# Ameek94/BOBE

Measured on AMD Instinct MI355X. Metric: GP fit+acquisition cycles/sec at N=4096 d=8, 65536 cands; Cholesky GF/s, higher is better.
Workload: dtype f64

## Files before the change

bobe_amd/csrc/chol_kernels.hpp:

```cpp
#pragma once
#include "kernels_common.hpp"

namespace bobe {

constexpr int PLD = 130;
constexpr int POTF2_DLD = 17;

template <bool LOWER = false, int NWAVES = 4>
__device__ __forceinline__ void block_load(double* S, const double* __restrict__ G, int64_t ld) {
  const int lane = threadIdx.x & 63, wave = threadIdx.x >> 6;
  constexpr int NI = TILE / NWAVES;
  v2d v[NI];
#pragma unroll
  for (int i = 0; i < NI; ++i) {
    const int r = NWAVES * i + wave;
    const int c = LOWER ? ((2 * lane <= r) ? 2 * lane : (r & ~1)) : 2 * lane;
    v[i] = *reinterpret_cast<const v2d*>(G + (int64_t)r * ld + c);
  }
#pragma unroll
  for (int i = 0; i < NI; ++i) *reinterpret_cast<v2d*>(S + (NWAVES * i + wave) * PLD + 2 * lane) = v[i];
}
__device__ __forceinline__ void block_store_lower(const double* S, double* __restrict__ G, int64_t ld) {
  const int lane = threadIdx.x & 63, wave = threadIdx.x >> 6;
#pragma unroll 8
// ... 305 lines not shown
          for (int ks = 0; ks < 4; ++ks) {
            const double av = S[(16 * i + (lane & 15)) * PLD + 16 * k + 4 * ks + (lane >> 4)];
            const double bv = S[(16 * k + 4 * ks + (lane >> 4)) * PLD + 16 * j + (lane & 15)];
            tacc = __builtin_amdgcn_mfma_f64_16x16x4f64(av, bv, tacc, 0, 0, 0);
          }
        }
        v4d racc = (v4d){0.0, 0.0, 0.0, 0.0};
#pragma unroll
        for (int r = 0; r < 4; ++r) {
          const double av = -S[(16 * i + (lane & 15)) * PLD + 16 * i + (lane >> 4) + 4 * r];
          racc = __builtin_amdgcn_mfma_f64_16x16x4f64(av, tacc[r], racc, 0, 0, 0);
        }
        if (slot == 0) res0 = racc; else res1 = racc;
      }
    }
    __syncthreads();
#pragma unroll
    for (int slot = 0; slot < 2; ++slot) {
      const int j = wave + 4 * slot;
      if (j < i) {
        const v4d racc = slot == 0 ? res0 : res1;
#pragma unroll
        for (int r = 0; r < 4; ++r) S[(16 * i + (lane >> 4) + 4 * r) * PLD + 16 * j + (lane & 15)] = racc[r];
      }
    }
    __syncthreads();
  }
  block_store_lower(S, Ib, ldl);
}

__global__ __launch_bounds__(256) void k_trti_diag(double* __restrict__ L, int64_t lda,
                                                   double* __restrict__ Linv, int64_t ldl, int64_t bsA = 0,
                                                   int64_t bsL = 0, const double* __restrict__ diag = nullptr,
                                                   int64_t bsD = 0, int first_aside = 1 << 30) {
  extern __shared__ double S[];
  const int blk = blockIdx.x;
  L += blockIdx.y * bsA;
  Linv += blockIdx.y * bsL;
  double* Lb = L + ((int64_t)blk * TILE) * lda + (int64_t)blk * TILE;
  double* Ib = Linv + ((int64_t)blk * TILE) * ldl + (int64_t)blk * TILE;
  if (diag && blk >= first_aside) {
    block_load(S, diag + blockIdx.y * bsD + (int64_t)blk * TILE * TILE, TILE);
    __syncthreads();
    block_store_lower(S, Lb, lda);
  } else {
    block_load(S, Lb, lda);
  }
  __syncthreads();
  trti_block(S, Ib, ldl);
}

constexpr int TRSM_DLD = 17;
constexpr int TRSM_SMEM_BYTES = (TILE * PLD + 8 * 16 * TRSM_DLD) * 8;
__global__ __launch_bounds__(256) void k_trsm_panel(double* __restrict__ A, int64_t lda,
                                                    const double* __restrict__ Dinv, int64_t ldl, int k,
                                                    int64_t bsA = 0, int64_t bsL = 0) {
  extern __shared__ double S[];
  A += blockIdx.y * bsA;
  Dinv += blockIdx.y * bsL;
  double* D = S + TILE * PLD;
  const int t = threadIdx.x, lane = t & 63, wave = t >> 6;
  const int64_t row0 = (int64_t)(k + 1) * TILE + (int64_t)blockIdx.x * 64 + wave * 16;
  const int64_t col0 = (int64_t)k * TILE;
  const double* Lkk = A + col0 * lda + col0;
  const double* Dk = Dinv + col0 * ldl + col0;
  const int g = lane >> 4, li = lane & 15;
  double* Aw = A + row0 * lda + col0;
  double* Sw = S + (wave * 16) * PLD;
  v2d xr[16], lr[32];
// ... 464 lines not shown
```

bobe_amd/csrc/gp_consumers.hip:

```cpp
#include "gp_handle.hpp"

#include "consumer_kernels.hpp"

using namespace bobe;

namespace bobe {
void configure_consumer_kernels() {
  static bool done[64] = {false};
  if (!first_use_on_device(done)) return;
  for_each_kern_dcap([](auto KE, auto DC) {
    allow_big_lds((k_hmc_run<KE, DC>), CHAIN_LDS_BYTES);
    allow_big_lds((k_rwalk<KE, DC>), CHAIN_LDS_BYTES);
    allow_big_lds((k_nuts_run<KE, DC>), NUTS_LDS_BYTES);
  });
}
}

void bobe_gp::set_gate(const double* sv, int64_t n_sv, const double* dual, double intercept, double gamma, double threshold,
                       double minus_inf) {
  use();
  sync();
  if (!sv || n_sv <= 0) {
    gate = Gate{nullptr, nullptr, 0, 0, 0.0, 0.0, threshold, minus_inf, GATE_NONE, nullptr, nullptr, 0.0, 0.0};
    return;
// ... 395 lines not shown
  not_pd = src.not_pd;
}

void bobe_gp::release_all() {
  (void)hipSetDevice(device);
  if (stream) (void)hipStreamSynchronize(stream);
  DBuf* bufs[] = {&X, &y, &XsT, &A, &Linv, &Tmp, &alpha, &w, &part, &gpart, &res, &info, &probs, &diag, &in_stage, &z_stage, &CsT, &ZsT, &kXC, &kXZ, &VZ, &WZ, &basez, &sc, &qpart, &pv,
                  &ps, &o_mean, &o_var, &o_wipv, &o_wipstd, &o_misc, &kin_a, &kin_b, &kout, &wg_ws, &gate_sv, &gate_dual, &gate_ell, &ell_ws, &ell_perm,
                  &vxc, &vxc2, &loo_ws};
  for (DBuf* b : bufs) b->release();
  for (auto& pr : prof_events) {
    (void)hipEventDestroy(pr.first);
    (void)hipEventDestroy(pr.second);
  }
  if (h_res) (void)hipHostFree(h_res);
  if (h_in) (void)hipHostFree(h_in);
  h_in = nullptr;
  for (hipStream_t st : slot_streams) {
    (void)hipStreamSynchronize(st);
    (void)hipStreamDestroy(st);
  }
  own.release();
  batch.release();
  for (EvalWs* sl : slots) {
    sl->release();
    delete sl;
  }
  slots.clear();
  for (auto& kv : chol_plans) {
    kv.second.d_jobs.release();
    kv.second.d_colk0.release();
  }
  if (ev_batch) (void)hipEventDestroy(ev_batch);
  if (own_stream && stream) (void)hipStreamDestroy(stream);
}
```

bobe_amd/csrc/gp_factor.hip:

```cpp
#include "gp_handle.hpp"

#include <chrono>

#include "chol_kernels.hpp"

using namespace bobe;

namespace bobe {

constexpr int SYRK32_BK = 128, SYRK64_BK = 16;
constexpr int SYRK32_SMEM = gemm_smem_doubles_exact<KC, KC, 32, 32, SYRK32_BK>() * 8 / 2;
constexpr int SYRK64_SMEM = gemm_smem_doubles_exact<KC, KC, 64, 64, SYRK64_BK>() * 8;

void configure_factor_kernels() {
  static bool done[64] = {false};
  if (!first_use_on_device(done)) return;
  allow_big_lds(k_potf2<true>, POTF2_SMEM_BYTES);
  allow_big_lds(k_potf2<false>, POTF2_SMEM_BYTES);
  allow_big_lds(k_trti_diag, POTF2_SMEM_BYTES);
  allow_big_lds(k_trsm_panel, TRSM_SMEM_BYTES);
  allow_big_lds((k_chol_panel<false, 3>), POTF2_SMEM_BYTES);
  allow_big_lds((k_chol_panel<false, 4>), POTF2_SMEM_BYTES);
  allow_big_lds((k_chol_panel<true, 3>), POTF2_SMEM_BYTES);
  allow_big_lds((k_chol_panel<true, 4>), POTF2_SMEM_BYTES);
  allow_big_lds(k_trtri_T<128>, GEMM_SMEM_BYTES);
  allow_big_lds(k_trtri_R<128>, GEMM_SMEM_BYTES);
  allow_big_lds(k_syrk_trail<64, SYRK64_BK>, SYRK64_SMEM);
  allow_big_lds(k_syrk_trail<64, SYRK64_BK, true>, SYRK64_SMEM);
  allow_big_lds(k_syrk_trail<32, SYRK32_BK>, SYRK32_SMEM);
  allow_big_lds(k_trtri_T<64>, GEMM64_SMEM_BYTES);
  allow_big_lds(k_trtri_R<64>, GEMM64_SMEM_BYTES);
  allow_big_lds(k_trtri_T<64, true>, GEMM64_SMEM_BYTES);
  allow_big_lds(k_trtri_R<64, true>, GEMM64_SMEM_BYTES);
  allow_big_lds(k_trtri_T<32>, GEMM32_SMEM_BYTES);
  allow_big_lds(k_trtri_R<32>, GEMM32_SMEM_BYTES);
  allow_big_lds(k_lauum_tiles32, GEMM32_SMEM_BYTES);
  for_each_kern_dcap([](auto KE, auto DC) {
    allow_big_lds((k_lauum_grad<KE, DC, 64>), GEMM64_SMEM_BYTES);
    allow_big_lds((k_lauum_grad<KE, DC, 64, true>), GEMM64_SMEM_BYTES);
    allow_big_lds((k_lauum_grad<KE, DC, 128>), GEMM_SMEM_BYTES);
  });
}

const Tuning& tuning() {
  static Tuning t = [] {
    Tuning v{512, 600, 300, 1, BOBE_MAX_MLL_SLOTS, 2048, 1, 1, false, false, true, true, true};
    auto geti = [](const char* name, int& dst) {
      const char* e = std::getenv(name);
      if (e) dst = std::atoi(e);
      return e != nullptr;
    };
    geti("BOBE_SYRK32_BELOW", v.syrk32_below);
    geti("BOBE_TRTRI64", v.trtri64_below);
    geti("BOBE_PAIR_MIN", v.pair_min);
    geti("BOBE_LOCKSTEP_MIN_N", v.lockstep_min_n);
    v.mll_slots_set = geti("BOBE_MLL_SLOTS", v.mll_slots);
    geti("BOBE_GRAPH_MAX_N", v.graph_max_n);
    geti("BOBE_XCD_SHARES", v.xcd_shares);
    geti("BOBE_FILL", v.fill);
    v.trace = std::getenv("BOBE_TRACE") != nullptr;
    int reuse = 1;
    geti("BOBE_FACTOR_REUSE", reuse);
    v.factor_reuse = reuse != 0;
    int glds = 1;
    geti("BOBE_GEMM_GLDS", glds);
    v.gemm_glds = glds != 0;
    int glds64 = 1;
    geti("BOBE_GEMM64_GLDS", glds64);
    v.gemm64_glds = glds64 != 0;
    return v;
  }();
  return t;
}

double default_refine_kappa() {
  static const double v = [] {
    const char* e = std::getenv("BOBE_REFINE_KAPPA");
    return e ? std::atof(e) : 1e6;
  }();
  return v;
}

int default_solve_block() {
  static const int v = [] {
    const char* e = std::getenv("BOBE_SOLVE_BLOCK");
    const int b = e ? std::atoi(e) : TILE;
    return b > 0 ? (b + TILE - 1) / TILE * TILE : TILE;
  }();
  return v;
}

int default_solve_panel() {
  static const int v = [] {
    const char* e = std::getenv("BOBE_SOLVE_PANEL");
    const int b = e ? std::atoi(e) : 512;
    return b > 0 ? (b + TILE - 1) / TILE * TILE : 512;
  }();
  return v;
}

int64_t default_solve_chunk() {
  static const int64_t v = [] {
    const char* e = std::getenv("BOBE_SOLVE_CHUNK");
    const int64_t c = e ? std::atoll(e) : 32768;
    return c > 0 ? (c + TILE - 1) / TILE * TILE : 0;
  }();
  return v;
}

double default_pivot_floor_ulp() {
  static const double v = [] {
    const char* e = std::getenv("BOBE_PIVOT_FLOOR_ULP");
    if (!e) return 0.0;
    const double u = std::atof(e);
    return u >= 0.0 ? u : 0.0;
  }();
  return v;
}

}

void bobe_gp::build_probs() {
  struct Item { int depth, lo, mid, hi; };
  std::vector<Item> items;
  struct Rec {
    static void go(std::vector<Item>& it, int depth, int lo, int hi) {
      if (hi - lo <= 1) return;
      const int mid = lo + (hi - lo) / 2;
      it.push_back({depth, lo, mid, hi});
      go(it, depth + 1, lo, mid);
      go(it, depth + 1, mid, hi);
    }
  };
  Rec::go(items, 0, 0, nb);
  int maxd = -1;
  for (auto& i : items) maxd = i.depth > maxd ? i.depth : maxd;
  std::vector<TriProb> flat;
  depths.clear();
  for (int dd = 0; dd <= maxd; ++dd) {
    Depth D{(int)flat.size(), 0, 0};
    for (auto& i : items)
      if (i.depth == dd) {
        flat.push_back({i.lo, i.mid, i.hi, D.nblocks});
        D.nblocks += (i.hi - i.mid) * (i.mid - i.lo);
        D.count++;
      }
    depths.push_back(D);
  }
  if (!flat.empty()) {
    probs.ensure(flat.size() * sizeof(TriProb));
    HIPCHK(hipMemcpy(probs.p, flat.data(), flat.size() * sizeof(TriProb), hipMemcpyHostToDevice));
  }
}

void bobe_gp::alloc_for_n() {
  own.ensure(*this, 1);
  const size_t mat = (size_t)Np * Np * sizeof(double);
  const size_t vec = (size_t)Np * sizeof(double);
  A.ensure(mat);
  Linv.ensure(mat);
  Tmp.ensure(mat);
  y.ensure(vec);
  alpha.ensure(vec);
  w.ensure(vec);
  XsT.ensure((size_t)d * vec);
  const int64_t pw = Np > chunk ? Np : chunk;
  part.ensure((size_t)nb * pw * sizeof(double));
  gpart.ensure((size_t)own.gps() * sizeof(double));
  res.ensure(128 * sizeof(double));
  info.ensure(sizeof(int));
  diag.ensure((size_t)nb * TILE * TILE * sizeof(double));
  build_probs();
  build_plans();
  forget_evals();
}

void bobe_gp::EvalWs::ensure(const bobe_gp& g, int B) {
  if (!h_res) {
    HIPCHK(hipHostMalloc(reinterpret_cast<void**>(&h_res), (size_t)width * (128 * sizeof(double) + sizeof(Hyper)),
                         hipHostMallocDefault));
    h_hyp = reinterpret_cast<Hyper*>(h_res + (size_t)width * 128);
  }
  if (B > cap || g.Np != Np) {
    for (bobe::EvalTag& t : tag) t.clear();
// ... 193 lines not shown
    for (int f = 1; f < nb; ++f) {
      const auto dc = build(f, nullptr);
      if (dc.first > 0 && dc.second * FILL_SLACK <= dc.first) { far = f; break; }
    }
  }
  CholPlan& pl = chol_plans[key];
  build(far, &pl);
  for (const FillJob& j : pl.jobs)
    if (!(j.ti >= j.tj && j.ti < 2 * nb && j.tj >= 0 && j.k0 >= 0 && j.k1 > j.k0 && j.k1 <= j.tj - (j.tj & 1)))
      throw Err(BOBE_ERR_STATE, "internal error: filler job outside the matrix");
  if (!pl.jobs.empty()) {
    pl.d_jobs.ensure(pl.jobs.size() * sizeof(FillJob));
    HIPCHK(hipMemcpy(pl.d_jobs.p, pl.jobs.data(), pl.jobs.size() * sizeof(FillJob), hipMemcpyHostToDevice));
  }
  bool need_tab = false;
  for (const CholOp& op : pl.ops) need_tab = need_tab || (op.kind != 0 && !op.uniform);
  if (need_tab) {
    pl.d_colk0.ensure(pl.colk0.size() * sizeof(int));
    HIPCHK(hipMemcpy(pl.d_colk0.p, pl.colk0.data(), pl.colk0.size() * sizeof(int), hipMemcpyHostToDevice));
  }
  if (tu.trace)
    std::fprintf(stderr, "[bobe] chol plan nb=%d B=%d fill=%d: deferred columns from %d, %lld of %lld tile-panels in fillers, "
                 "%lld caught up (%zu jobs)\n", nb, B, (int)fill, pl.far_start, (long long)pl.deferred_units,
                 (long long)pl.total_units, (long long)pl.catchup_units, pl.jobs.size());
  return pl;
}

void bobe_gp::build_plans() {
  if (nb <= 0) return;
  (void)chol_plan(1, false);
  if (fill_pays(1)) (void)chol_plan(1, true);
}

void bobe_gp::potrf(double* a, double* linv, int* info_dev, int B, int64_t bsA, int64_t bsL, double* dg, bool defer_diag) {
  if (!dg) dg = diag.d();
  const int64_t bsD = (int64_t)nb * TILE * TILE;
  int first_aside = nb;
  const CholPlan& pl = chol_plan(B, fill_pays(B));
  const FillJob* jobs = static_cast<const FillJob*>(pl.d_jobs.p);
  const int* coltab = static_cast<const int*>(pl.d_colk0.p);
  for (const CholOp& op : pl.ops) {
    if (op.kind == 0) {
      const int kk = op.k;
      const int rr = nb - 1 - kk;
      const int strips = panel_strips(B, rr);
      const int np_ = panel_workgroups(rr, strips);
      const int rows_below = rr * TILE;
      const int nv = (int)std::min<int64_t>(TILE, N - (int64_t)kk * TILE);
      if (B * np_ <= std::max(num_cus, 1)) {
        first_aside = std::min(first_aside, kk);
        prof_begin(BOBE_PROF_POTF2);
#define PANEL_LAUNCH(FILLV, GRIDX, ...)                                                                                        \
  do {                                                                                                                         \
    if (strips == 3)                                                                                                           \
      hipLaunchKernelGGL((k_chol_panel<FILLV, 3>), dim3(GRIDX, B), dim3(PANEL_THREADS), POTF2_SMEM_BYTES, stream, a, Np, bsA, \
                         linv, Np, bsL, kk, np_, info_dev, nv, dg, bsD, __VA_ARGS__);                                          \
    else                                                                                                                       \
      hipLaunchKernelGGL((k_chol_panel<FILLV, 4>), dim3(GRIDX, B), dim3(PANEL_THREADS), POTF2_SMEM_BYTES, stream, a, Np, bsA, \
                         linv, Np, bsL, kk, np_, info_dev, nv, dg, bsD, __VA_ARGS__);                                          \
  } while (0)
        if (op.tab_cnt > 0) PANEL_LAUNCH(true, np_ + op.tab_cnt / 2, jobs + op.tab_off, op.tab_cnt, rows_below);
        else PANEL_LAUNCH(false, np_, (const FillJob*)nullptr, 0, rows_below);
#undef PANEL_LAUNCH
        prof_end(BOBE_PROF_POTF2);
      } else {
        prof_begin(BOBE_PROF_POTF2);
        hipLaunchKernelGGL(k_potf2<true>, dim3(B), dim3(256), POTF2_SMEM_BYTES, stream, a, Np, linv, Np, kk, info_dev, nv, bsA,
                           bsL);
        prof_end(BOBE_PROF_POTF2);
        if (rr > 0) {
          prof_begin(BOBE_PROF_TRSM);
          hipLaunchKernelGGL(k_trsm_panel, dim3(2 * rr, B), dim3(256), TRSM_SMEM_BYTES, stream, a, Np, (const double*)linv, Np,
                             kk, bsA, bsL);
          prof_end(BOBE_PROF_TRSM);
        }
      }
    } else {
      prof_begin(BOBE_PROF_SYRK);
      if (op.uniform) {
        syrk(a, op.k0_min, op.k, op.first, op.kind == 1 ? 1 : 0, B, bsA);
      } else {
        const int ncols = op.last_active - op.first + 1;
        const bool few = ncols <= 8 && ncols < nb - op.first;
        syrk(a, op.k0_plain, op.k, op.first, few ? 2 : 0, B, bsA, coltab + op.tab_off, pl.far_start, few ? ncols : 0);
      }
      prof_end(BOBE_PROF_SYRK);
    }
  }
  cur->aside_first = 1 << 30;
  cur->aside_dg = nullptr;
  if (first_aside < nb) {
    if (defer_diag) {
      cur->aside_first = first_aside;
      cur->aside_dg = dg;
    } else {
      hipLaunchKernelGGL(k_copy_diag, dim3(nb - first_aside, B), dim3(256), 0, stream, a, Np, bsA, (const double*)dg, bsD,
                         first_aside);
    }
  }
  LAUNCH_CHECK();
}

void bobe_gp::trtri(double* a, double* linv, double* tmp, int B, int64_t bsA, int64_t bsL, int64_t bsT) {
  const Tuning& tu = tuning();
  prof_begin(BOBE_PROF_TRTRI);
  hipLaunchKernelGGL(k_trti_diag, dim3(nb, B), dim3(256), POTF2_SMEM_BYTES, stream, a, Np, linv, Np, bsA, bsL, cur->aside_dg,
                     (int64_t)nb * TILE * TILE, cur->aside_first);
  cur->aside_first = 1 << 30;
  cur->aside_dg = nullptr;
  prof_end(BOBE_PROF_TRTRI);
  for (int dd = (int)depths.size() - 1; dd >= 0; --dd) {
    const Depth& D = depths[dd];
    const TriProb* pr = static_cast<const TriProb*>(probs.p) + D.first;
    prof_begin(BOBE_PROF_TRTRI);
    if (B * 2 * D.nblocks <= std::max(num_cus, 1)) {
      const TileGrid tg = tile_grid(8 * D.nblocks);
      hipLaunchKernelGGL(k_trtri_T<32>, dim3(tg.grid, B), dim3(256), GEMM32_SMEM_BYTES, stream, a, Np,
                         (const double*)linv, Np, tmp, Np, pr, D.count, bsA, bsL, bsT, tg.per);
      hipLaunchKernelGGL(k_trtri_R<32>, dim3(tg.grid, B), dim3(256), GEMM32_SMEM_BYTES, stream, linv, Np,
                         (const double*)tmp, Np, pr, D.count, bsL, bsT, tg.per);
    } else if (D.nblocks < tu.trtri64_below) {
      const TileGrid tg = tile_grid(2 * D.nblocks);
      const auto kT = tu.gemm64_glds ? k_trtri_T<64, true> : k_trtri_T<64, false>;
      const auto kR = tu.gemm64_glds ? k_trtri_R<64, true> : k_trtri_R<64, false>;
      hipLaunchKernelGGL(kT, dim3(tg.grid, B), dim3(256), GEMM64_SMEM_BYTES, stream, a, Np,
                         (const double*)linv, Np, tmp, Np, pr, D.count, bsA, bsL, bsT, tg.per);
      hipLaunchKernelGGL(kR, dim3(tg.grid, B), dim3(256), GEMM64_SMEM_BYTES, stream, linv, Np,
                         (const double*)tmp, Np, pr, D.count, bsL, bsT, tg.per);
    } else {
      hipLaunchKernelGGL(k_trtri_T<128>, dim3(D.nblocks, B), dim3(256), GEMM_SMEM_BYTES, stream, a, Np,
                         (const double*)linv, Np, tmp, Np, pr, D.count, bsA, bsL, bsT);
      hipLaunchKernelGGL(k_trtri_R<128>, dim3(D.nblocks, B), dim3(256), GEMM_SMEM_BYTES, stream, linv, Np,
                         (const double*)tmp, Np, pr, D.count, bsL, bsT);
    }
    prof_end(BOBE_PROF_TRTRI);
  }
  LAUNCH_CHECK();
}

int bobe_gp::lauum(const Hyper& h, const double* linv, const double* al, const double* xst, double* kinv_out,
                   const Hyper* hdev, double* gp_out, int B, int64_t bsL, int64_t bsV, int64_t bsX, int64_t bsP,
                   double* scratch, int64_t bsS, int64_t bsKout) {
  const LauumTiling t = lauum_tiling(nb);
  const int ntiles = t.ntiles;
  double* gpo = gp_out ? gp_out : gpart.d();
  const bool split = t.small && scratch && !kinv_out && B * ntiles < 4 * std::max(num_cus, 1);
  double* kio = split ? scratch : kinv_out;
  const int64_t bsK = split ? bsS : bsKout;
  prof_begin(BOBE_PROF_LAUUM);
  if (split) {
    hipLaunchKernelGGL(k_lauum_tiles32, dim3(4 * ntiles * B), dim3(256), GEMM32_SMEM_BYTES, stream, linv, Np, Np, scratch, Np,
                       bsL, bsS, B);
  }
  with_lauum_variant(h.kern, h.d, t, [&](auto KE, auto DC, auto TT, auto GL) {
    hipLaunchKernelGGL((k_lauum_grad<KE, DC, TT, GL>), dim3(ntiles * B), dim3(256),
                       (TT == 128 ? GEMM_SMEM_BYTES : GEMM64_SMEM_BYTES), stream, linv, Np, Np, N, al, xst, Np, h, gpo, kio,
                       Np, hdev, bsL, bsV, bsX, bsP, B, split ? 1 : 0, bsK);
  });
  prof_end(BOBE_PROF_LAUUM);
  LAUNCH_CHECK();
  return ntiles;
}

void bobe_gp::solve_alpha(const double* linv, double* wv, double* al, double* prt, int B, int64_t bsL, int64_t bsV,
                          int64_t bsP, const double* rhs, int64_t bsY) {
  hipLaunchKernelGGL(k_gemv_lower, dim3((unsigned)(Np / 4), (unsigned)B), dim3(256), 0, stream, linv, Np, Np,
                     rhs ? rhs : (const double*)y.d(), wv, bsL, bsV, rhs ? bsY : (int64_t)0);
  hipLaunchKernelGGL(k_gemv_t_part, dim3((unsigned)(Np / 64), (unsigned)nb, (unsigned)B), dim3(256), 0, stream, linv, Np, 1,
                     (const double*)wv, prt, Np, bsL, bsV, bsP);
  hipLaunchKernelGGL(k_colsum_parts, dim3((unsigned)((Np + 255) / 256), (unsigned)B), dim3(256), 0, stream,
                     (const double*)prt, Np, nb, 1, Np, al, bsP, bsV);
  LAUNCH_CHECK();
}

void bobe_gp::chol_solve(const FactorBufs& f, int B, const double* rhs) {
  potrf(f.a, f.linv, f.info, B, f.mat, f.mat, f.diag, true);
  trtri(f.a, f.linv, f.tmp, B, f.mat, f.mat, f.mat);
  solve_alpha(f.linv, f.w, f.alpha, f.part, B, f.mat, f.vec, f.prt, rhs, 0);
}

void bobe_gp::factor_into(const Hyper& h, const FactorBufs& f, const Hyper* hdev, int B) {
  scale(X.d(), N, Np, h, f.xst, Np, hdev, B, f.xs, f.info);
  assemble_kxx(h, f.xst, f.a, hdev, B, f.xs, f.mat);
  chol_solve(f, B);
}

void bobe_gp::mll_terms(const double* wv, const double* a, double* res_dev, const int* info_dev) {
  hipLaunchKernelGGL(k_mll_terms, dim3(1), dim3(256), 0, stream, wv, a, Np, Np, res_dev, (int64_t)0, (int64_t)0, (int64_t)0,
                     info_dev);
  LAUNCH_CHECK();
}

void bobe_gp::res_to_host(const double* res_dev, double* h, int n) {
  HIPCHK(hipMemcpyAsync(h, res_dev, (size_t)n * sizeof(double), hipMemcpyDeviceToHost, stream));
  sync();
}

std::string bobe_gp::not_pd_text(int inf, double min_diag) const {
  if (inf != 0x7f7f7f7f) return "kernel matrix not positive definite at column " + std::to_string(inf - 1);
  char buf[200];
  if (min_diag != min_diag)
    std::snprintf(buf, sizeof buf, "kernel matrix not positive definite: NaN pivot");
  else
    std::snprintf(buf, sizeof buf,
                  "kernel matrix numerically singular: smallest pivot %.3g is below %g ulp of its diagonal (rank test)",
                  min_diag * min_diag, pivot_ulp);
  return buf;
}

const std::vector<hipStream_t>& bobe_gp::slot_stream_set() {
// ... 34 lines not shown
  const int64_t gps = ws.stride(ws.gps()), rs = ws.stride(128);
  if (hdev) HIPCHK(hipMemcpyAsync(ws.hyp.p, ws.h_hyp, (size_t)B * sizeof(Hyper), hipMemcpyHostToDevice, stream));
  factor_into(hs[0], f, hdev, B);
  if (want_grad) {
    const int ntiles = lauum(hs[0], f.linv, f.alpha, f.xst, nullptr, hdev, ws.gpart.d(), B, f.mat, f.vec, f.xs, gps, f.tmp,
                             f.mat);
    hipLaunchKernelGGL(k_mll_grad_reduce, dim3(d + 2, B), dim3(256), 0, stream, (const double*)ws.gpart.d(), ntiles,
                       dcap_of(d) + 1, d, dcap_of(d), ws.res.d(), (const double*)f.w, (const double*)f.a, Np, Np,
                       (const int*)f.info, gps, rs, f.vec, f.mat);
    if (noise_grad) mll_noise_tail(ws, B, hs, hdev);
  } else {
    hipLaunchKernelGGL(k_mll_terms, dim3(B), dim3(256), 0, stream, (const double*)f.w, (const double*)f.a, Np, Np, ws.res.d(),
                       f.vec, f.mat, rs, (const int*)f.info);
  }
  LAUNCH_CHECK();
  HIPCHK(hipMemcpyAsync(ws.h_res, ws.res.p, (size_t)(ws.width > 1 ? B * 128 : 102) * sizeof(double), hipMemcpyDeviceToHost,
                        stream));
}

void bobe_gp::eval_replay(EvalWs& ws, const Hyper* hs, bool want_grad) {
  EvalGraph& eg = ws.eg;
  const int w = want_grad ? 1 : 0;
  const std::array<const void*, 16> sig = {ws.XsT.p, ws.A.p, ws.Linv.p, ws.Tmp.p, ws.w.p, ws.alpha.p, ws.part.p, ws.gpart.p,
                                           ws.res.p, ws.info.p, X.p, y.p, probs.p, static_cast<const void*>(ws.h_res),
                                           reinterpret_cast<const void*>(static_cast<uintptr_t>(N)),
                                           static_cast<const void*>(stream)};
  if (!eg.exec[w] || eg.sig[w] != sig) {
    if (eg.exec[w]) {
      (void)hipGraphExecDestroy(eg.exec[w]);
      eg.exec[w] = nullptr;
    }
    hipGraph_t graph = nullptr;
    HIPCHK(hipStreamBeginCapture(stream, hipStreamCaptureModeThreadLocal));
    try {
      eval_enqueue(ws, 1, hs, want_grad, static_cast<const Hyper*>(ws.hyp.p));
    } catch (...) {
      (void)hipStreamEndCapture(stream, &graph);
      if (graph) (void)hipGraphDestroy(graph);
      throw;
    }
    HIPCHK(hipStreamEndCapture(stream, &graph));
    const hipError_t ie = hipGraphInstantiate(&eg.exec[w], graph, nullptr, nullptr, 0);
    (void)hipGraphDestroy(graph);
    if (ie != hipSuccess) {
      eg.exec[w] = nullptr;
      HIPCHK(ie);
    }
    eg.sig[w] = sig;
  }
  HIPCHK(hipGraphLaunch(eg.exec[w], stream));
}

void bobe_gp::eval_start(EvalWs& ws, int B, const Hyper* hs, bool want_grad, bool noise_grad) {
  noise_grad = noise_grad && want_grad;
  UseWs use_ws(*this, ws);
  for (int b = 0; b < B; ++b) {
    ws.tag[b].clear();
    ws.h_hyp[b] = hs[b];
    ws.floor[b] = pivot_floor(hs[b]);
  }
  if (ws.width > 1) eval_enqueue(ws, B, hs, want_grad, static_cast<const Hyper*>(ws.hyp.p), noise_grad);
  else if (noise_grad || !on_slot() || N > tuning().graph_max_n || prof_tag != 0)
    eval_enqueue(ws, 1, hs, want_grad, nullptr, noise_grad);
  else eval_replay(ws, hs, want_grad);
  for (int b = 0; b < B; ++b) ws.tag[b].arm(hs[b], data_gen, Np);
}

int bobe_gp::eval_result(const double* hr, double floor, double* mll, double* grad, bool noise_grad) const {
  const int ng = d + 1 + (noise_grad ? 1 : 0);
  int inf;
  std::memcpy(&inf, hr + 100, sizeof(int));
  if (inf != 0x7f7f7f7f || !pivots_resolved(hr[101], floor)) {
    *mll = std::nan("");
// ... 464 lines not shown
```

bobe_amd/csrc/gp_handle.hpp:

```cpp
#pragma once
#include "../../include/bobe_gp.h"

#include <hip/hip_runtime.h>

#include <algorithm>
#include <array>
#include <climits>
#include <cmath>
#include <cstdio>
#include <cstdlib>
#include <cstring>
#include <map>
#include <mutex>
#include <stdexcept>
#include <string>
#include <type_traits>
#include <vector>

#include "gemm_f64.hpp"
#include "gp_types.hpp"

namespace bobe {

struct Err : std::runtime_error {
  int code;
  Err(int c, const std::string& m) : std::runtime_error(m), code(c) {}
};

extern thread_local std::string g_err;

#define HIPCHK(expr)                                                                                           \
  do {                                                                                                         \
    hipError_t e_ = (expr);                                                                                    \
    if (e_ != hipSuccess)                                                                                      \
      throw ::bobe::Err(BOBE_ERR_HIP, std::string(#expr) + ": " + hipGetErrorString(e_) + " (" __FILE__ ":" + \
                                          std::to_string(__LINE__) + ")");                                     \
  } while (0)

#define LAUNCH_CHECK() HIPCHK(hipGetLastError())

inline int64_t round_up(int64_t x, int64_t m) { return (x + m - 1) / m * m; }

inline bool is_device_ptr(const void* p) {
  if (!p) return false;
// ... 19 lines not shown
  }
  void release() {
    if (p) (void)hipFree(p);
    p = nullptr;
    bytes = 0;
  }
  double* d() const { return static_cast<double*>(p); }
};

struct CallBuf : DBuf {
  CallBuf() = default;
  CallBuf(const CallBuf&) = delete;
  CallBuf& operator=(const CallBuf&) = delete;
  ~CallBuf() { release(); }
};

inline double pivot_floor(const Hyper& h, double ulp) {
  const double f = ulp * 2.220446049250313e-16 * (h.kvar + h.noise);
  return f < 0.25 ? f : 0.25;
}
inline bool pivots_resolved(double min_diag, double floor) { return min_diag * min_diag >= floor; }
double default_pivot_floor_ulp();
double default_refine_kappa();
int default_solve_block();
int default_solve_panel();
int64_t default_solve_chunk();

template <typename K>
void allow_big_lds(K kernel, int bytes) {
  HIPCHK(hipFuncSetAttribute(reinterpret_cast<const void*>(kernel), hipFuncAttributeMaxDynamicSharedMemorySize, bytes));
}

struct Tuning {
  int syrk32_below, trtri64_below, pair_min, lockstep_min_n, mll_slots, graph_max_n, xcd_shares, fill;
  bool mll_slots_set, trace, factor_reuse, gemm_glds, gemm64_glds;
};
const Tuning& tuning();

inline int dcap_of(int d) { return d <= 8 ? 8 : (d <= 16 ? 16 : 32); }
template <typename F>
inline void with_dcap(int d, F&& f) {
  switch (dcap_of(d)) {
    case 8: f(std::integral_constant<int, 8>{}); break;
    case 16: f(std::integral_constant<int, 16>{}); break;
    default: f(std::integral_constant<int, 32>{}); break;
  }
}
template <typename F>
inline void with_kern_dcap(int kern, int d, F&& f) {
  with_dcap(d, [&](auto DC) {
    if (kern == 0) f(std::integral_constant<int, 0>{}, DC);
    else f(std::integral_constant<int, 1>{}, DC);
  });
}
template <typename F>
inline void for_each_kern_dcap(F&& f) {
  for (int kern = 0; kern < 2; ++kern)
    for (int d : {8, 16, 32}) with_kern_dcap(kern, d, f);
}

constexpr int LAUUM64_BELOW = 1200;
struct LauumTiling { bool small; int nt, ntiles; };
inline LauumTiling lauum_tiling(int nb) {
  const bool small = nb * (nb + 1) / 2 < LAUUM64_BELOW;
  const int nt = small ? 2 * nb : nb;
  return {small, nt, nt * (nt + 1) / 2};
}
template <typename F>
inline void with_lauum_variant(int kern, int d, const LauumTiling& t, F&& f) {
  with_kern_dcap(kern, d, [&](auto KE, auto DC) {
    if (!t.small) f(KE, DC, std::integral_constant<int, 128>{}, std::false_type{});
    else if (tuning().gemm64_glds) f(KE, DC, std::integral_constant<int, 64>{}, std::true_type{});
    else f(KE, DC, std::integral_constant<int, 64>{}, std::false_type{});
  });
}

constexpr int FILL_NEAR = 2;
constexpr int FILL_CHUNK = 3;
constexpr int FILL_SLACK = 16;
constexpr int FILL_PHASE = 1024;

struct TileGrid { int grid, per; };
inline TileGrid tile_grid(int ntiles) {
  if (!tuning().xcd_shares || ntiles < 256) return {ntiles, 0};
  const int per = (ntiles + 7) / 8;
  return {8 * per, per};
}

void configure_factor_kernels();
void configure_sweep_kernels();
void configure_consumer_kernels();
void configure_posterior_kernels();
void configure_loo_kernels();
void configure_paths_kernels();
inline bool first_use_on_device(bool (&done)[64]) {
  int dev = 0;
  HIPCHK(hipGetDevice(&dev));
  if (dev < 0 || dev >= 64 || done[dev]) return false;
  return done[dev] = true;
}

struct Depth { int first, count, nblocks; };

struct SweepKeep {
  double* CsT = nullptr;
  double* V = nullptr;
  double* crossT = nullptr;
  double* sc = nullptr;
  int64_t ld = 0;
  const double* V_used = nullptr;
  int64_t ldv_used = 0;
};

struct SweepW {
  const double* logw = nullptr;
  double* out[4] = {nullptr, nullptr, nullptr, nullptr};
  CallBuf zt, zpart, lstage;
  int64_t ldt = 0;
  double* log_s() const { return zt.d() + (int64_t)ZTERM_ROWS * ldt; }
};

struct SweepReq {
  const double* cand = nullptr;
  int64_t C = 0;
  const double* Z = nullptr;
  int64_t M = 0;
  double y_std = 1.0;
  double* wipv = nullptr;
  double* wipstd = nullptr;
  double* mean = nullptr;
  double* var = nullptr;
  int policy = 1;
  int64_t* argmin_v = nullptr;
  double* min_v = nullptr;
  int64_t* argmin_s = nullptr;
// ... 41 lines not shown
  typedef bobe::Hyper Hyper;
  int device = 0;
  int kern = 0;
  int d = 0;
  hipStream_t stream = nullptr;
  bool own_stream = false;
  int64_t N = 0, Np = 0;
  int nb = 0;
  Hyper hyp;
  uint64_t data_gen = 0;
  double pivot_ulp = bobe::default_pivot_floor_ulp();
  double pivot_floor(const Hyper& h) const { return bobe::pivot_floor(h, pivot_ulp); }
  bool have_data = false, factored = false, not_pd = false;
  double refine_kappa = bobe::default_refine_kappa();
  bool refine_v = false;
  int solve_block = bobe::default_solve_block();
  int solve_panel = bobe::default_solve_panel();
  int64_t solve_chunk = bobe::default_solve_chunk();
  void decide_refinement(double min_diag);
  void solve_v(double* B, int64_t ldb, int64_t ncp, double* V, int64_t ldv, double* qp, int64_t ldq);
  void solve_wt(const double* V, int64_t ldv, int64_t ncp, double* W, int64_t ldw);
  std::vector<double> z_seen;
  int64_t z_seen_m = -1;
  bool wz_ready = false;
  void forget_z() { z_seen_m = -1; wz_ready = false; }
  int64_t chunk = 8192;
  bool chunk_set = false;

  DBuf X, y, XsT, A, Linv, Tmp, alpha, w, part, gpart, res, info, probs, diag;
  int num_cus = 0;
  DBuf wg_ws;
  DBuf in_stage, z_stage, CsT, ZsT, kXC, kXZ, VZ, WZ, basez, sc, qpart, pv, ps, o_mean, o_var, o_wipv, o_wipstd,
      o_misc, kin_a, kin_b, kout, vxc, vxc2;
  std::vector<bobe::Depth> depths;
  double* h_res = nullptr;
  double* h_in = nullptr;

  DBuf gate_sv, gate_dual, gate_ell;
  bobe::Gate gate{nullptr, nullptr, 0, 0, 0.0, 0.0, 0.5, -1e5};
  void set_gate(const double* sv, int64_t n_sv, const double* dual, double intercept, double gamma, double threshold,
                double minus_inf);
  void set_gate_ellipsoid(const double* flat_L, const double* mu, double alpha, double beta, double threshold,
                          double minus_inf);
  DBuf ell_ws, ell_perm;
  void train_ellipsoid(const double* X, const double* y, int64_t N, const double* mu, int n_restarts, const double* init,
                       const int32_t* perm, int n_epochs, int batch, double lr, double wd, double* params_out,
                       double* loss_out);
  void gate_apply(const double* xq_dev, int64_t C, double* decision, double* feasible, double* mean, double* var,
                  double* dmean, double* dvar, double* proba = nullptr);
  void gate_eval(const double* Xq, int64_t C, double* decision, double* feasible);
  void gate_proba(const double* Xq, int64_t C, double* proba);

  struct CholOp {
    int kind;
    int k;
    int first;
    int tab_off, tab_cnt;
    int k0_min, k0_max;
    bool uniform;
    int last_active;
    int k0_plain;
  };
  struct CholPlan {
    std::vector<CholOp> ops;
    std::vector<bobe::FillJob> jobs;
    std::vector<int> colk0;
    DBuf d_jobs, d_colk0;
// ... 116 lines not shown
  }
  void sync() { HIPCHK(hipStreamSynchronize(stream)); }

  const double* fetch(const double* p, size_t n, DBuf& stage) {
    if (bobe::is_device_ptr(p)) return p;
    stage.ensure(n * sizeof(double));
    HIPCHK(hipMemcpyAsync(stage.p, p, n * sizeof(double), hipMemcpyHostToDevice, stream));
    return stage.d();
  }
  double* out_dev(double* user, size_t n, DBuf& stage) {
    if (!user) return nullptr;
    if (bobe::is_device_ptr(user)) return user;
    stage.ensure(n * sizeof(double));
    return stage.d();
  }
  void out_finish(double* user, size_t n, DBuf& stage) {
    if (!user || bobe::is_device_ptr(user)) return;
    HIPCHK(hipMemcpyAsync(user, stage.p, n * sizeof(double), hipMemcpyDeviceToHost, stream));
  }

  void build_probs();
  void alloc_for_n();
  void set_data(const double* X, const double* ys, int64_t N);
  void scale(const double* in, int64_t n, int64_t npad, const Hyper& h, double* out, int64_t ldo,
             const Hyper* hdev = nullptr, int B = 1, int64_t bsO = 0, int* info_reset = nullptr);
  void kernel_matrix_cross(const double* AT, int64_t lda, int64_t na, int64_t napad, const double* BT, int64_t ldb,
                           int64_t nbv, int64_t nbpad, const Hyper& h, double* out, int64_t ldo,
                           const double* wv = nullptr, double* prt = nullptr, int64_t ldp = 0);
  void assemble_kxx(const Hyper& h, const double* xst, double* a, const Hyper* hdev = nullptr, int B = 1,
                    int64_t bsX = 0, int64_t bsA = 0);
  void syrk(double* a, int k0, int k1, int first, int colmode, int B = 1, int64_t bsA = 0, const int* colk0 = nullptr,
            int far_col = 0, int ncols = 0);
  void potrf(double* a, double* linv, int* info_dev, int B = 1, int64_t bsA = 0, int64_t bsL = 0, double* dg = nullptr,
             bool defer_diag = false);
  void trtri(double* a, double* linv, double* tmp, int B = 1, int64_t bsA = 0, int64_t bsL = 0, int64_t bsT = 0);
  int lauum(const Hyper& h, const double* linv, const double* al, const double* xst, double* kinv_out,
            const Hyper* hdev = nullptr, double* gp_out = nullptr, int B = 1, int64_t bsL = 0, int64_t bsV = 0,
            int64_t bsX = 0, int64_t bsP = 0, double* scratch = nullptr, int64_t bsS = 0, int64_t bsK = 0);
  void solve_alpha(const double* linv, double* wv, double* al, double* prt, int B = 1, int64_t bsL = 0, int64_t bsV = 0,
                   int64_t bsP = 0, const double* rhs = nullptr, int64_t bsY = 0);
  void factor_into(const Hyper& h, const FactorBufs& f, const Hyper* hdev = nullptr, int B = 1);
  void chol_solve(const FactorBufs& f, int B = 1, const double* rhs = nullptr);
  void mll_terms(const double* wv, const double* a, double* res_dev, const int* info_dev);
  void res_to_host(const double* res_dev, double* h, int n);
  std::string not_pd_text(int inf, double min_diag) const;
  void size_workspace(int64_t n);
  int mll_from_k(const double* K, int64_t n, const double* yv, double* mll);
  void chol_row_update(const double* L, int64_t n, const double* k, double k_self, double* v, double* diag_out);
  int factor_state();
  void forget_evals();
  const bobe::EvalTag* adopt_factor();
  int factor_source = -1;
  void copy_out_matrix(const double* src, double* dst, int lower_only);
  void get_chol(double* L, double* alpha_out);
  void set_chol(const double* L, const double* alpha_in);
  double min_pivot_root();
  void kinv_debug(double* Kinv);
  double time_potrf(int reps);
  double time_potrf_batch(int B, int reps);
  double time_potrf_lockstep(int B, int reps);
  double time_potrf_wide(EvalWs& ws, int B, int reps);
  void fill(double* p, int64_t n, double v);

  void prepare_z(const double* Z, int64_t M, int64_t Mp, bool need_w);
  void wip_score(const double* crossT, int64_t ldx, const double* cst, const double* scs, const double* bz, int64_t ns,
                 int64_t M, int64_t Mp, double y_std, double* wv, double* ws, double* vo);
  void sweep(const bobe::SweepReq& r);
  void wip_grad(const double* cand, int64_t C, const double* Z, int64_t M, double y_std, double* wipv, double* wipstd,
// ... 59 lines not shown
```

bobe_amd/csrc/gp_types.hpp:

```cpp
#pragma once
#include <hip/hip_runtime.h>
#include <stdint.h>

namespace bobe {

constexpr int MAX_D = 32;
constexpr int ZTERM_ROWS = 5;

struct Hyper {
  double ls[MAX_D];
  double kvar;
  double noise;
  int d;
  int kern;
};

struct TriProb { int lo, mid, hi, off; };

enum { FILL_TWIN = 1 };
struct FillJob { int ti, tj, k0, k1, flags, pad0; };

enum GateKind { GATE_NONE = 0, GATE_SVM = 1, GATE_ELLIPSOID = 2 };
struct Gate {
  const double* svT;
  const double* dual;
  int64_t ld;
  int n_sv;
  double intercept, gamma, threshold, minus_inf;
  int kind;
  const double* Lt;
  const double* mu;
  double alpha, beta;
};
__host__ __device__ inline bool gate_on(const Gate& g) { return g.kind != GATE_NONE; }

}
```

Before: 19.79.

## Overlap leading-half triangular inverse with remaining Cholesky on a side stream

Splits the recursive triangular inversion into a leading half, a trailing half and a top-level combine. Once the factorisation has finished the panels of the leading half, that half's inverse is launched on a second stream masked to three quarters of the CUs, so it runs alongside the rest of the potrf. The trailing part then runs on the main stream, which joins on the side stream before the final combine step. This hides the serial chain of small trtri launches behind the factorisation, at the cost of extra streams and events, contention for CUs, and a heuristic gate that skips the path during graph capture and for large problems.

```diff
diff --git a/bobe_amd/csrc/chol_kernels.hpp b/bobe_amd/csrc/chol_kernels.hpp
--- a/bobe_amd/csrc/chol_kernels.hpp
+++ b/bobe_amd/csrc/chol_kernels.hpp
@@ -361,9 +361,9 @@
 __global__ __launch_bounds__(256) void k_trti_diag(double* __restrict__ L, int64_t lda,
                                                    double* __restrict__ Linv, int64_t ldl, int64_t bsA = 0,
                                                    int64_t bsL = 0, const double* __restrict__ diag = nullptr,
-                                                   int64_t bsD = 0, int first_aside = 1 << 30) {
+                                                   int64_t bsD = 0, int first_aside = 1 << 30, int blk0 = 0) {
   extern __shared__ double S[];
-  const int blk = blockIdx.x;
+  const int blk = blk0 + blockIdx.x;
   L += blockIdx.y * bsA;
   Linv += blockIdx.y * bsL;
   double* Lb = L + ((int64_t)blk * TILE) * lda + (int64_t)blk * TILE;
diff --git a/bobe_amd/csrc/gp_consumers.hip b/bobe_amd/csrc/gp_consumers.hip
--- a/bobe_amd/csrc/gp_consumers.hip
+++ b/bobe_amd/csrc/gp_consumers.hip
@@ -451,5 +451,11 @@
     kv.second.d_colk0.release();
   }
   if (ev_batch) (void)hipEventDestroy(ev_batch);
+  if (side_stream) {
+    (void)hipStreamSynchronize(side_stream);
+    (void)hipStreamDestroy(side_stream);
+  }
+  if (ev_fork) (void)hipEventDestroy(ev_fork);
+  if (ev_join) (void)hipEventDestroy(ev_join);
   if (own_stream && stream) (void)hipStreamDestroy(stream);
 }
diff --git a/bobe_amd/csrc/gp_factor.hip b/bobe_amd/csrc/gp_factor.hip
--- a/bobe_amd/csrc/gp_factor.hip
+++ b/bobe_amd/csrc/gp_factor.hip
@@ -44,7 +44,7 @@
 
 const Tuning& tuning() {
   static Tuning t = [] {
-    Tuning v{512, 600, 300, 1, BOBE_MAX_MLL_SLOTS, 2048, 1, 1, false, false, true, true, true};
+    Tuning v{512, 600, 300, 1, BOBE_MAX_MLL_SLOTS, 2048, 1, 1, 1, false, false, true, true, true};
     auto geti = [](const char* name, int& dst) {
       const char* e = std::getenv(name);
       if (e) dst = std::atoi(e);
@@ -58,6 +58,7 @@
     geti("BOBE_GRAPH_MAX_N", v.graph_max_n);
     geti("BOBE_XCD_SHARES", v.xcd_shares);
     geti("BOBE_FILL", v.fill);
+    geti("BOBE_INV_SIDE", v.inv_side);
     v.trace = std::getenv("BOBE_TRACE") != nullptr;
     int reuse = 1;
     geti("BOBE_FACTOR_REUSE", reuse);
@@ -121,35 +122,14 @@
 }
 
 void bobe_gp::build_probs() {
-  struct Item { int depth, lo, mid, hi; };
-  std::vector<Item> items;
-  struct Rec {
-    static void go(std::vector<Item>& it, int depth, int lo, int hi) {
-      if (hi - lo <= 1) return;
-      const int mid = lo + (hi - lo) / 2;
-      it.push_back({depth, lo, mid, hi});
-      go(it, depth + 1, lo, mid);
-      go(it, depth + 1, mid, hi);
-    }
-  };
-  Rec::go(items, 0, 0, nb);
-  int maxd = -1;
-  for (auto& i : items) maxd = i.depth > maxd ? i.depth : maxd;
-  std::vector<TriProb> flat;
-  depths.clear();
-  for (int dd = 0; dd <= maxd; ++dd) {
-    Depth D{(int)flat.size(), 0, 0};
-    for (auto& i : items)
-      if (i.depth == dd) {
-        flat.push_back({i.lo, i.mid, i.hi, D.nblocks});
-        D.nblocks += (i.hi - i.mid) * (i.mid - i.lo);
-        D.count++;
-      }
-    depths.push_back(D);
-  }
-  if (!flat.empty()) {
-    probs.ensure(flat.size() * sizeof(TriProb));
-    HIPCHK(hipMemcpy(probs.p, flat.data(), flat.size() * sizeof(TriProb), hipMemcpyHostToDevice));
+  const TriSplit sp = tri_split(nb);
+  depths = sp.depths;
+  lead_depths = sp.lead;
+  trail_depths = sp.trail;
+  tri_mid = sp.mid;
+  if (!sp.table.empty()) {
+    probs.ensure(sp.table.size() * sizeof(TriProb));
+    HIPCHK(hipMemcpy(probs.p, sp.table.data(), sp.table.size() * sizeof(TriProb), hipMemcpyHostToDevice));
   }
 }
 
@@ -409,7 +389,8 @@
   if (fill_pays(1)) (void)chol_plan(1, true);
 }
 
-void bobe_gp::potrf(double* a, double* linv, int* info_dev, int B, int64_t bsA, int64_t bsL, double* dg, bool defer_diag) {
+void bobe_gp::potrf(double* a, double* linv, int* info_dev, int B, int64_t bsA, int64_t bsL, double* dg, bool defer_diag,
+                    const std::function<void(int)>* at_fork, int fork_panel) {
   if (!dg) dg = diag.d();
   const int64_t bsD = (int64_t)nb * TILE * TILE;
   int first_aside = nb;
@@ -452,6 +433,7 @@
           prof_end(BOBE_PROF_TRSM);
         }
       }
+      if (at_fork && kk == fork_panel) (*at_fork)(first_aside);
     } else {
       prof_begin(BOBE_PROF_SYRK);
       if (op.uniform) {
@@ -478,41 +460,64 @@
   LAUNCH_CHECK();
 }
 
+void bobe_gp::trtri_level(const TriArgs& t, const Depth& part, int level_blocks, bool do_t, bool do_r) {
+  const Tuning& tu = tuning();
+  const TriProb* pr = static_cast<const TriProb*>(probs.p) + part.first;
+  if (t.B * 2 * level_blocks <= std::max(num_cus, 1)) {
+    const TileGrid tg = tile_grid(8 * part.nblocks);
+    if (do_t)
+      hipLaunchKernelGGL(k_trtri_T<32>, dim3(tg.grid, t.B), dim3(256), GEMM32_SMEM_BYTES, stream, t.a, Np,
+                         (const double*)t.linv, Np, t.tmp, Np, pr, part.count, t.bsA, t.bsL, t.bsT, tg.per);
+    if (do_r)
+      hipLaunchKernelGGL(k_trtri_R<32>, dim3(tg.grid, t.B), dim3(256), GEMM32_SMEM_BYTES, stream, t.linv, Np,
+                         (const double*)t.tmp, Np, pr, part.count, t.bsL, t.bsT, tg.per);
+  } else if (level_blocks < tu.trtri64_below) {
+    const TileGrid tg = tile_grid(2 * part.nblocks);
+    const auto kT = tu.gemm64_glds ? k_trtri_T<64, true> : k_trtri_T<64, false>;
+    const auto kR = tu.gemm64_glds ? k_trtri_R<64, true> : k_trtri_R<64, false>;
+    if (do_t)
+      hipLaunchKernelGGL(kT, dim3(tg.grid, t.B), dim3(256), GEMM64_SMEM_BYTES, stream, t.a, Np, (const double*)t.linv, Np,
+                         t.tmp, Np, pr, part.count, t.bsA, t.bsL, t.bsT, tg.per);
+    if (do_r)
+      hipLaunchKernelGGL(kR, dim3(tg.grid, t.B), dim3(256), GEMM64_SMEM_BYTES, stream, t.linv, Np, (const double*)t.tmp, Np,
+                         pr, part.count, t.bsL, t.bsT, tg.per);
+  } else {
+    if (do_t)
+      hipLaunchKernelGGL(k_trtri_T<128>, dim3(part.nblocks, t.B), dim3(256), GEMM_SMEM_BYTES, stream, t.a, Np,
+                         (const double*)t.linv, Np, t.tmp, Np, pr, part.count, t.bsA, t.bsL, t.bsT);
+    if (do_r)
+      hipLaunchKernelGGL(k_trtri_R<128>, dim3(part.nblocks, t.B), dim3(256), GEMM_SMEM_BYTES, stream, t.linv, Np,
+                         (const double*)t.tmp, Np, pr, part.count, t.bsL, t.bsT);
+  }
+}
+
+void bobe_gp::trtri_part(TriPart part, const TriArgs& t, const double* dg, int first_aside) {
+  const int b0 = part == TRI_TRAIL ? tri_mid : 0, b1 = part == TRI_LEAD ? tri_mid : nb;
+  if (part != TRI_TOP_R) {
+    prof_begin(BOBE_PROF_TRTRI);
+    hipLaunchKernelGGL(k_trti_diag, dim3(b1 - b0, t.B), dim3(256), POTF2_SMEM_BYTES, stream, t.a, Np, t.linv, Np, t.bsA, t.bsL,
+                       dg, (int64_t)nb * TILE * TILE, first_aside, b0);
+    prof_end(BOBE_PROF_TRTRI);
+  }
+  for (int dd = (int)depths.size() - 1; dd >= 0; --dd) {
+    const Depth& D = depths[dd];
+    if (part != TRI_ALL && dd > 0) {
+      const Depth& P = part == TRI_LEAD ? lead_depths[dd] : trail_depths[dd];
+      if (part != TRI_TOP_R && P.count > 0) trtri_level(t, P, D.nblocks, true, true);
+      continue;
+    }
+    if (part == TRI_TRAIL) continue;
+    prof_begin(BOBE_PROF_TRTRI);
+    trtri_level(t, D, D.nblocks, part != TRI_TOP_R, part != TRI_LEAD);
+    prof_end(BOBE_PROF_TRTRI);
+  }
+  LAUNCH_CHECK();
+}
+
 void bobe_gp::trtri(double* a, double* linv, double* tmp, int B, int64_t bsA, int64_t bsL, int64_t bsT) {
-  const Tuning& tu = tuning();
-  prof_begin(BOBE_PROF_TRTRI);
-  hipLaunchKernelGGL(k_trti_diag, dim3(nb, B), dim3(256), POTF2_SMEM_BYTES, stream, a, Np, linv, Np, bsA, bsL, cur->aside_dg,
-                     (int64_t)nb * TILE * TILE, cur->aside_first);
+  trtri_part(TRI_ALL, {a, linv, tmp, B, bsA, bsL, bsT}, cur->aside_dg, cur->aside_first);
   cur->aside_first = 1 << 30;
   cur->aside_dg = nullptr;
-  prof_end(BOBE_PROF_TRTRI);
-  for (int dd = (int)depths.size() - 1; dd >= 0; --dd) {
-    const Depth& D = depths[dd];
-    const TriProb* pr = static_cast<const TriProb*>(probs.p) + D.first;
-    prof_begin(BOBE_PROF_TRTRI);
-    if (B * 2 * D.nblocks <= std::max(num_cus, 1)) {
-      const TileGrid tg = tile_grid(8 * D.nblocks);
-      hipLaunchKernelGGL(k_trtri_T<32>, dim3(tg.grid, B), dim3(256), GEMM32_SMEM_BYTES, stream, a, Np,
-                         (const double*)linv, Np, tmp, Np, pr, D.count, bsA, bsL, bsT, tg.per);
-      hipLaunchKernelGGL(k_trtri_R<32>, dim3(tg.grid, B), dim3(256), GEMM32_SMEM_BYTES, stream, linv, Np,
-                         (const double*)tmp, Np, pr, D.count, bsL, bsT, tg.per);
-    } else if (D.nblocks < tu.trtri64_below) {
-      const TileGrid tg = tile_grid(2 * D.nblocks);
-      const auto kT = tu.gemm64_glds ? k_trtri_T<64, true> : k_trtri_T<64, false>;
-      const auto kR = tu.gemm64_glds ? k_trtri_R<64, true> : k_trtri_R<64, false>;
-      hipLaunchKernelGGL(kT, dim3(tg.grid, B), dim3(256), GEMM64_SMEM_BYTES, stream, a, Np,
-                         (const double*)linv, Np, tmp, Np, pr, D.count, bsA, bsL, bsT, tg.per);
-      hipLaunchKernelGGL(kR, dim3(tg.grid, B), dim3(256), GEMM64_SMEM_BYTES, stream, linv, Np,
-                         (const double*)tmp, Np, pr, D.count, bsL, bsT, tg.per);
-    } else {
-      hipLaunchKernelGGL(k_trtri_T<128>, dim3(D.nblocks, B), dim3(256), GEMM_SMEM_BYTES, stream, a, Np,
-                         (const double*)linv, Np, tmp, Np, pr, D.count, bsA, bsL, bsT);
-      hipLaunchKernelGGL(k_trtri_R<128>, dim3(D.nblocks, B), dim3(256), GEMM_SMEM_BYTES, stream, linv, Np,
-                         (const double*)tmp, Np, pr, D.count, bsL, bsT);
-    }
-    prof_end(BOBE_PROF_TRTRI);
-  }
-  LAUNCH_CHECK();
 }
 
 int bobe_gp::lauum(const Hyper& h, const double* linv, const double* al, const double* xst, double* kinv_out,
@@ -550,9 +555,67 @@
   LAUNCH_CHECK();
 }
 
+bool bobe_gp::inv_side_pays(int B) const {
+  const int f = tuning().inv_side;
+  if (f == 0 || nb < 2 || on_slot() || capturing || prof_tag == BOBE_PROF_TRTRI) return false;
+  if (f == 2) return true;
+  return nb >= 16 && (int64_t)B * nb * nb * nb <= 900000;
+}
+
+void bobe_gp::ensure_side() {
+  if (side_stream) return;
+  if (!ev_fork) HIPCHK(hipEventCreateWithFlags(&ev_fork, hipEventDisableTiming));
+  if (!ev_join) HIPCHK(hipEventCreateWithFlags(&ev_join, hipEventDisableTiming));
+  const int words = (num_cus + 31) / 32;
+  std::vector<uint32_t> mask(words, 0u);
+  for (int c = 0; c < 3 * num_cus / 4; ++c) mask[c / 32] |= (1u << (c % 32));
+  hipStream_t st = nullptr;
+  if (num_cus < 4 || hipExtStreamCreateWithCUMask(&st, (uint32_t)words, mask.data()) != hipSuccess) {
+    (void)hipGetLastError();
+    st = nullptr;
+  }
+  if (!st) HIPCHK(hipStreamCreateWithFlags(&st, hipStreamNonBlocking));
+  side_stream = st;
+}
+
 void bobe_gp::chol_solve(const FactorBufs& f, int B, const double* rhs) {
-  potrf(f.a, f.linv, f.info, B, f.mat, f.mat, f.diag, true);
-  trtri(f.a, f.linv, f.tmp, B, f.mat, f.mat, f.mat);
+  const TriArgs t{f.a, f.linv, f.tmp, B, f.mat, f.mat, f.mat};
+  if (inv_side_pays(B)) {
+    ensure_side();
+    struct Join {
+      bobe_gp& g;
+      bool forked = false, joined = false;
+      ~Join() {
+        if (forked && !joined) (void)hipStreamSynchronize(g.side_stream);
+      }
+    } join{*this};
+    const std::function<void(int)> fork = [&](int first_aside) {
+      HIPCHK(hipEventRecord(ev_fork, stream));
+      HIPCHK(hipStreamWaitEvent(side_stream, ev_fork, 0));
+      join.forked = true;
+      {
+        struct OnSide {
+          bobe_gp& g;
+          const hipStream_t main;
+          ~OnSide() { g.stream = main; }
+        } on_side{*this, stream};
+        stream = side_stream;
+        trtri_part(TRI_LEAD, t, f.diag, first_aside);
+      }
+      HIPCHK(hipEventRecord(ev_join, side_stream));
+    };
+    potrf(f.a, f.linv, f.info, B, f.mat, f.mat, f.diag, true, &fork, tri_mid - 1);
+    if (!join.forked) throw Err(BOBE_ERR_STATE, "internal error: the factorisation has no panel to fork the inverse after");
+    trtri_part(TRI_TRAIL, t, cur->aside_dg, cur->aside_first);
+    cur->aside_first = 1 << 30;
+    cur->aside_dg = nullptr;
+    HIPCHK(hipStreamWaitEvent(stream, ev_join, 0));
+    join.joined = true;
+    trtri_part(TRI_TOP_R, t, nullptr, 0);
+  } else {
+    potrf(f.a, f.linv, f.info, B, f.mat, f.mat, f.diag, true);
+    trtri(f.a, f.linv, f.tmp, B, f.mat, f.mat, f.mat);
+  }
   solve_alpha(f.linv, f.w, f.alpha, f.part, B, f.mat, f.vec, f.prt, rhs, 0);
 }
 
@@ -653,13 +716,16 @@
     }
     hipGraph_t graph = nullptr;
     HIPCHK(hipStreamBeginCapture(stream, hipStreamCaptureModeThreadLocal));
+    capturing = true;
     try {
       eval_enqueue(ws, 1, hs, want_grad, static_cast<const Hyper*>(ws.hyp.p));
     } catch (...) {
+      capturing = false;
       (void)hipStreamEndCapture(stream, &graph);
       if (graph) (void)hipGraphDestroy(graph);
       throw;
     }
+    capturing = false;
     HIPCHK(hipStreamEndCapture(stream, &graph));
     const hipError_t ie = hipGraphInstantiate(&eg.exec[w], graph, nullptr, nullptr, 0);
     (void)hipGraphDestroy(graph);
diff --git a/bobe_amd/csrc/gp_handle.hpp b/bobe_amd/csrc/gp_handle.hpp
--- a/bobe_amd/csrc/gp_handle.hpp
+++ b/bobe_amd/csrc/gp_handle.hpp
@@ -10,6 +10,7 @@
 #include <cstdio>
 #include <cstdlib>
 #include <cstring>
+#include <functional>
 #include <map>
 #include <mutex>
 #include <stdexcept>
@@ -95,7 +96,7 @@
 }
 
 struct Tuning {
-  int syrk32_below, trtri64_below, pair_min, lockstep_min_n, mll_slots, graph_max_n, xcd_shares, fill;
+  int syrk32_below, trtri64_below, pair_min, lockstep_min_n, mll_slots, graph_max_n, xcd_shares, fill, inv_side;
   bool mll_slots_set, trace, factor_reuse, gemm_glds, gemm64_glds;
 };
 const Tuning& tuning();
@@ -162,8 +163,6 @@
   if (dev < 0 || dev >= 64 || done[dev]) return false;
   return done[dev] = true;
 }
-
-struct Depth { int first, count, nblocks; };
 
 struct SweepKeep {
   double* CsT = nullptr;
@@ -271,7 +270,8 @@
   DBuf wg_ws;
   DBuf in_stage, z_stage, CsT, ZsT, kXC, kXZ, VZ, WZ, basez, sc, qpart, pv, ps, o_mean, o_var, o_wipv, o_wipstd,
       o_misc, kin_a, kin_b, kout, vxc, vxc2;
-  std::vector<bobe::Depth> depths;
+  std::vector<bobe::Depth> depths, lead_depths, trail_depths;
+  int tri_mid = 0;
   double* h_res = nullptr;
   double* h_in = nullptr;
 
@@ -454,8 +454,21 @@
   void syrk(double* a, int k0, int k1, int first, int colmode, int B = 1, int64_t bsA = 0, const int* colk0 = nullptr,
             int far_col = 0, int ncols = 0);
   void potrf(double* a, double* linv, int* info_dev, int B = 1, int64_t bsA = 0, int64_t bsL = 0, double* dg = nullptr,
-             bool defer_diag = false);
+             bool defer_diag = false, const std::function<void(int)>* at_fork = nullptr, int fork_panel = -1);
+  struct TriArgs {
+    double *a, *linv, *tmp;
+    int B;
+    int64_t bsA, bsL, bsT;
+  };
+  enum TriPart { TRI_ALL, TRI_LEAD, TRI_TRAIL, TRI_TOP_R };
+  void trtri_part(TriPart part, const TriArgs& t, const double* dg, int first_aside);
+  void trtri_level(const TriArgs& t, const bobe::Depth& part, int level_blocks, bool do_t, bool do_r);
   void trtri(double* a, double* linv, double* tmp, int B = 1, int64_t bsA = 0, int64_t bsL = 0, int64_t bsT = 0);
+  hipStream_t side_stream = nullptr;
+  hipEvent_t ev_fork = nullptr, ev_join = nullptr;
+  bool capturing = false;
+  bool inv_side_pays(int B) const;
+  void ensure_side();
   int lauum(const Hyper& h, const double* linv, const double* al, const double* xst, double* kinv_out,
             const Hyper* hdev = nullptr, double* gp_out = nullptr, int B = 1, int64_t bsL = 0, int64_t bsV = 0,
             int64_t bsX = 0, int64_t bsP = 0, double* scratch = nullptr, int64_t bsS = 0, int64_t bsK = 0);
diff --git a/bobe_amd/csrc/gp_types.hpp b/bobe_amd/csrc/gp_types.hpp
--- a/bobe_amd/csrc/gp_types.hpp
+++ b/bobe_amd/csrc/gp_types.hpp
@@ -1,6 +1,8 @@
 #pragma once
 #include <hip/hip_runtime.h>
 #include <stdint.h>
+
+#include "tri_split.hpp"
 
 namespace bobe {
 
@@ -15,7 +17,6 @@
   int kern;
 };
 
-struct TriProb { int lo, mid, hi, off; };
 
 enum { FILL_TWIN = 1 };
 struct FillJob { int ti, tj, k0, k1, flags, pad0; };
diff --git a/bobe_amd/csrc/tri_split.hpp b/bobe_amd/csrc/tri_split.hpp
--- /dev/null
+++ b/bobe_amd/csrc/tri_split.hpp
@@ -0,0 +1,64 @@
+#pragma once
+#include <vector>
+
+namespace bobe {
+
+struct TriProb { int lo, mid, hi, off; };
+
+struct Depth { int first, count, nblocks; };
+
+struct TriSplit {
+  std::vector<TriProb> table;
+  std::vector<Depth> depths, lead, trail;
+  int mid = 0;
+};
+
+inline TriSplit tri_split(int nb) {
+  struct Item { int depth, lo, mid, hi; };
+  std::vector<Item> items;
+  struct Rec {
+    static void go(std::vector<Item>& it, int depth, int lo, int hi) {
+      if (hi - lo <= 1) return;
+      const int mid = lo + (hi - lo) / 2;
+      it.push_back({depth, lo, mid, hi});
+      go(it, depth + 1, lo, mid);
+      go(it, depth + 1, mid, hi);
+    }
+  };
+  Rec::go(items, 0, 0, nb);
+  TriSplit s;
+  s.mid = nb >= 2 ? nb / 2 : 0;
+  int maxd = -1;
+  for (auto& i : items) maxd = i.depth > maxd ? i.depth : maxd;
+  for (int dd = 0; dd <= maxd; ++dd) {
+    Depth D{(int)s.table.size(), 0, 0}, Ld{D.first, 0, 0};
+    for (auto& i : items)
+      if (i.depth == dd) {
+        const int blocks = (i.hi - i.mid) * (i.mid - i.lo);
+        s.table.push_back({i.lo, i.mid, i.hi, D.nblocks});
+        D.nblocks += blocks;
+        D.count++;
+        if (dd > 0 && i.hi <= s.mid) {
+          Ld.nblocks += blocks;
+          Ld.count++;
+        }
+      }
+    s.depths.push_back(D);
+    s.lead.push_back(Ld);
+  }
+  for (int dd = 0; dd <= maxd; ++dd) {
+    const Depth D = s.depths[dd], Ld = s.lead[dd];
+    Depth Td{(int)s.table.size(), 0, 0};
+    for (int q = D.first + Ld.count; dd > 0 && q < D.first + D.count; ++q) {
+      TriProb p = s.table[q];
+      p.off -= Ld.nblocks;
+      s.table.push_back(p);
+      Td.nblocks += (p.hi - p.mid) * (p.mid - p.lo);
+      Td.count++;
+    }
+    s.trail.push_back(Td);
+  }
+  return s;
+}
+
+}
```

Result: faster. 20.38 (median of 6 runs) (+3.0%).
